# frozenreboot/rplidar_ros2_driver

Measured on AMD Instinct MI355X. Metric: Mpoints/s raw-scan->filtered PointCloud2, higher is better.
Workload: dtype u32/f32

## Files before the change

### rplidar_ros2_driver_amd/csrc/rpl_launch.hpp

```cpp
#pragma once
#include <hip/hip_runtime.h>
#include <stdint.h>

#include "rplgpu.h"
#include "rplgpu_msg.h"
#include "rplgpu_comm.h"
#include "rpl_device.hpp"
#include "rpl_msg.hpp"

namespace rplmsg {
struct Prefix;
}

namespace rpl {

constexpr uint32_t kAscendUnsorted = 0x80000000u;
constexpr uint32_t kRorListedBit = 0x80000000u;
constexpr uint32_t kScanStatusBits =
    RPLGPU_SCAN_ALL_INVALID | RPLGPU_SCAN_CELL_RANGE | RPLGPU_SCAN_TABLE_FULL | RPLGPU_SCAN_OUT_TRUNCATED;
static_assert((kAscendUnsorted & kScanStatusBits) == 0, "internal ascend bit overlaps RPLGPU_SCAN_*");
static_assert((kRorListedBit & kScanStatusBits) == 0, "internal cloud bit overlaps RPLGPU_SCAN_*");
hipError_t launch_ascend(hipStream_t s, void *nodes, uint32_t n_stride, const uint32_t *n_per_scan,
                         uint32_t B, uint32_t *status, uint32_t *need_sort, bool defer_sort = false,
                         uint32_t *sort_stat = nullptr);
hipError_t launch_ascend_sort(hipStream_t s, void *nodes, uint32_t n_stride, const uint32_t *n_per_scan,
                              uint32_t B, uint32_t *status, uint32_t *need_sort,
                              uint32_t *sort_stat = nullptr);
struct LsMsgOut {
  rplmsg::Prefix P;
  uint32_t *msg;
  uint32_t *msg_len;
  int32_t sec;
  uint32_t nanosec;
  double scan_duration;
};
hipError_t launch_laserscan_a(hipStream_t s, const void *nodes, uint32_t n_stride,
                              const uint32_t *n_per_scan, uint32_t B, const KParams &p,
                              const Tables &T, const float *inc_table, const float *rinc_table,
                              bool fast, float *ranges, float *intens, uint32_t *beam_count,
                              uint32_t n_given = 0xFFFFFFFFu, const LsMsgOut *msg_out = nullptr);
hipError_t launch_validate_idx(hipStream_t s, const Tables &T, const float *inc_table,
                               const float *rinc_table, uint32_t max_count,
                               uint32_t *d_mismatches);
hipError_t launch_laserscan_raw(hipStream_t s, const void *nodes, uint32_t n_stride,
                                const uint32_t *n_per_scan, uint32_t B, const KParams &p,
                                float *ranges, float *intens, uint32_t *beam_count);
hipError_t launch_cloud(hipStream_t s, const void *nodes, uint32_t n_stride,
                        const uint32_t *n_per_scan, uint32_t B, const KParams &p, const Tables &T,
                        const uint32_t *keepmask, uint32_t mask_stride, float *xyzi,
                        uint32_t out_stride, uint32_t *n_points, uint32_t *status,
                        const float *motion = nullptr);
enum class ArenaForm : int { kXyzi = 0, kXyi = 1, kCells = 2 };
enum class RorMode : int { kNone = 0, kInside = 1, kListed = 2 };
struct VoxelLaunch {
  const void *nodes = nullptr;
  uint32_t n_stride = 0;
  const uint32_t *n_per_scan = nullptr;
  uint32_t B = 0;
  uint32_t group = 1;
  const float *motion = nullptr, *pose2d = nullptr;
  const uint32_t *keepmask = nullptr;
  uint32_t mask_stride = 0;
  RorMode ror = RorMode::kNone;
  float *xyzi = nullptr;
  uint32_t out_stride = 0;
  float *arena = nullptr;
  uint64_t arena_capacity = 0;
  uint64_t *arena_cursor = nullptr, *scan_start = nullptr;
  ArenaForm form = ArenaForm::kXyzi;
  uint32_t *n_points = nullptr, *status = nullptr;
};
hipError_t launch_cloud_voxel(hipStream_t s, const VoxelLaunch &v, const KParams &p, const Tables &T);
uint32_t voxel_max_workgroups(uint32_t n_cu);
inline uint64_t voxel_store_need(uint32_t group, uint32_t n_stride) {
  const uint64_t s = n_stride < kMaxN ? n_stride : kMaxN;
  return (uint64_t)(group ? group : 1u) * (s + 2u * ((s + 123u) / 124u) + 1u + 528u);
}
hipError_t launch_ror_mask(hipStream_t s, const void *nodes, uint32_t n_stride,
                           const uint32_t *n_per_scan, uint32_t B, const KParams &p,
                           const Tables &T, uint32_t *mask, uint32_t mask_stride,
                           bool listed = false, uint32_t group = 1);
hipError_t launch_validate_div(hipStream_t s, float d, float rd, uint32_t e_lo, uint32_t e_hi,
                               uint32_t *d_mismatches);
hipError_t launch_pack(hipStream_t s, const float *xyzi, uint32_t out_stride,
                       const uint32_t *n_points, uint32_t B, float *packed, uint64_t *offsets);

hipError_t launch_laserscan_to_cloud(hipStream_t s, const float *ranges, const float *intens,
                                     uint32_t n_stride, const uint32_t *beam_count, uint32_t B,
                                     const KParams &p, float *xyzi, uint32_t out_stride,
                                     uint32_t *n_points, uint32_t *status);

hipError_t launch_signal(hipStream_t s, uint32_t *flag, uint32_t seq);
hipError_t launch_stage_in(hipStream_t s, const void *src, void *dst, uint32_t n_words2);
hipError_t launch_pack_meta(hipStream_t s, const unsigned long long *cursor,
                            const unsigned long long *scan_start, const uint32_t *n_points,
                            uint32_t B, unsigned long long slot_points, uint32_t max_scans,
                            uint32_t *meta);
hipError_t launch_unpack_gathered(hipStream_t s, const float *points_all,
                                  unsigned long long slot_points, const uint32_t *meta_all,
                                  uint32_t meta_words, uint32_t world, uint32_t max_scans,
                                  float *packed, unsigned long long *total,
                                  unsigned long long *scan_start_all, uint32_t *n_points_all,
                                  uint32_t *status, uint32_t n_cu, bool xyi = false);
hipError_t launch_merge_cells(hipStream_t s, const void *cells_all, unsigned long long slot_cells,
                              const uint32_t *meta_all, uint32_t meta_words, uint32_t world,
                              uint32_t n_groups, double unit, float *arena,
                              unsigned long long capacity, unsigned long long *cursor,
                              unsigned long long *group_start, uint32_t *n_points, uint32_t *status,
                              uint32_t *scratch, uint32_t n_cu);
hipError_t launch_pack_xyi(hipStream_t s, const float *arena, const unsigned long long *cursor,
                           unsigned long long slot_points, float *slot, uint32_t n_cu);

hipError_t launch_decode(hipStream_t s, int ans, const uint8_t *bytes, uint64_t stream_stride,
                         const uint32_t *frame_off, const uint8_t *gap, const uint32_t *n_frames,
                         uint32_t max_frames, uint32_t B, uint32_t sample_duration_us,
                         const int32_t *state_in, int32_t *state_out, void *nodes,
                         uint32_t node_stride, uint32_t *n_nodes, uint32_t *reset_at,
                         uint32_t reset_stride, uint32_t *n_reset, uint32_t *n_errors,
                         uint32_t *status, uint32_t *sync_at = nullptr, uint32_t sync_stride = 0,
                         uint32_t *n_sync = nullptr, const uint32_t *only = nullptr,
                         bool staged_ok = true, uint32_t *stage_todo = nullptr);
// ... 151 lines not shown
```

### rplidar_ros2_driver_amd/csrc/rpl_voxel.hip

```cpp
#include <algorithm>
#include <cstdlib>
#include <type_traits>

#include "rpl_device.hpp"
#include "rpl_launch.hpp"
#include "rpl_xf.hpp"

namespace rpl {

#ifndef RPL_VOXEL_THREADS
#define RPL_VOXEL_THREADS 1024
#endif
#ifndef RPL_VOXEL_WGS_PER_CU
#define RPL_VOXEL_WGS_PER_CU (RPL_VOXEL_THREADS == 512 ? 2 : 1)
#endif
constexpr int kVB = RPL_VOXEL_THREADS;
constexpr int kVW = kVB / 64;
constexpr int kVWG = RPL_VOXEL_WGS_PER_CU;
constexpr uint32_t kRecCap = kVWG == 2 ? 4096u : 7168u;
constexpr uint32_t kRecPerThread = kRecCap / kVB;
constexpr uint32_t kRowCap = kVWG == 2 ? 1024u : 2u * kVB;
constexpr uint32_t kRowsPerThread = kRowCap / kVB;
constexpr uint32_t kBucketCap = kRecCap + 3u * kRowCap;
constexpr uint32_t kEmptyKey = 0xFFFFFFFFu;
// ... 242 lines not shown
  const u32x4 marker = {kEmptyKey, 0u, 0u, 0u};
  VoxelLds &L = S.L;
  uint4 *const G = S.G;
  const uint32_t lds_rec = (uint32_t)(uintptr_t)&L.rec[0];
  if (base + 1u + total <= kRecCap) {
    if (lane_id() == 0) lds_store128(lds_rec + base * 16u, marker);
#pragma unroll
    for (int j = 0; j < NS; ++j)
      if (__builtin_amdgcn_inverse_ballot_w64(m[j])) lds_store128(lds_rec + pos[j] * 16u, rec[j]);
  } else {
    if (lane_id() == 0) {
      if (base < kRecCap) lds_store128(lds_rec + base * 16u, marker); else glb_store128(G + base, marker);
    }
#pragma unroll
    for (int j = 0; j < NS; ++j) {
      if (__builtin_amdgcn_inverse_ballot_w64(m[j])) {
        if (pos[j] < kRecCap) lds_store128(lds_rec + pos[j] * 16u, rec[j]); else glb_store128(G + pos[j], rec[j]);
      }
    }
  }
  return false;
}

template <int NS>
__device__ __forceinline__ void voxel_block_split(QueueSink &S,
                                                  const bool (&ok)[NS], const uint32_t (&key)[NS],
                                                  const uint32_t (&qx)[NS], const uint32_t (&qy)[NS],
                                                  const uint32_t (&ci)[NS]) {
#pragma unroll
  for (uint32_t cls = 0; cls < 2u; ++cls) {
    bool okc[NS];
    uint32_t keyc[NS], qxc[NS], qyc[NS], cic[NS];
#pragma unroll
    for (int j = 0; j < NS; ++j) {
      okc[j] = ok[j] && (((key[j] >> 16) ^ key[j]) & 1u) == cls;
      keyc[j] = key[j];
      qxc[j] = okc[j] ? qx[j] : 0u;
      qyc[j] = okc[j] ? qy[j] : 0u;
      cic[j] = okc[j] ? ci[j] : 0u;
    }
    voxel_block_pass<true, NS, kPassPlain>(S, okc, keyc, qxc, qyc, cic);
  }
}

__device__ __forceinline__ double run_sum_f64(uint32_t u) {
  double s = (double)u;
  if (u >= 0xF0000000u) s -= 4294967296.0;
  return s;
}

struct VoxelArena {
  float4 *base;
  unsigned long long *cursor;
  unsigned long long capacity;
  unsigned long long *scan_start;
  int xyi;
};
enum : int { kEmitLegacy = 0, kEmitArenaFirst = 1, kEmitCountOnly = 2, kEmitArenaKnown = 3, kEmitArenaTemp = 4 };

template <bool DBG>
struct PhaseClock {
  unsigned long long acc[8] = {0, 0, 0, 0, 0, 0, 0, 0}, mark = 0;
  __device__ __forceinline__ void start() {
    if (DBG) mark = clock64();
  }
  __device__ __forceinline__ void lap(int i) {
    if (DBG) {
      const unsigned long long now = clock64();
      acc[i] += now - mark;
      mark = now;
    }
  }
};

template <bool DBG, bool CELLS>
__device__ __forceinline__ uint32_t voxel_reduce(VoxelLds &L, const KParams &p,
                                                 float4 *__restrict__ out, uint32_t out_stride,
                                                 uint32_t b, uint32_t *ncell_out, int mode,
                                                 const VoxelArena &arena, bool normalised,
                                                 const float4 *out_buffer) {
  PhaseClock<DBG> pc;
  pc.start();
  auto flush_dbg = [&]() {
    if (DBG && p.dbg && threadIdx.x == 0) {
#pragma unroll
      for (int i = 1; i < 8; ++i) atomicAdd(&p.dbg[16 * b + i], pc.acc[i]);
    }
  };
  uint32_t *const rowstart = L.rows, *const rowfill = L.rows + kRowCap;
  uint32_t *cell_keys = p.cell_keys ? p.cell_keys + (out - out_buffer) : nullptr;
  const int vbias = p.vox_bias;
  const uint32_t nrec = L.misc[0];
  if (DBG && p.dbg && threadIdx.x == 0) pc.acc[7] += (unsigned long long)nrec << 40;
  uint4 mine[kRecPerThread];
  uint32_t rmin = 0xFFFFFFFFu, rmax = 0u;
#pragma unroll
  for (int k = 0; k < (int)kRecPerThread; ++k) {
    const uint32_t idx = threadIdx.x + (uint32_t)k * kVB;
    uint4 m = make_uint4(kEmptyKey, 0u, 0u, 0u);
    if ((idx & ~63u) < nrec) {
      const uint4 raw = L.rec[idx];
      const bool ok = idx < nrec && raw.x != kEmptyKey;
      m = raw;
      if (!normalised) {
        uint4 pr;
        pr.y = (uint32_t)__builtin_amdgcn_update_dpp(0, (int)raw.y, 0x138, 0xF, 0xF, false);
// ... 480 lines not shown
  return false;
}

template <bool FAST_DIV, bool SAFE, bool SPLIT, bool DBG, int AHEAD, int RORM = 0>
__device__ __forceinline__ void voxel_stream_dispatch(QueueSink &sink, const KParams &p,
                                                      const float2 *__restrict__ cs,
                                                      const __amdgpu_buffer_rsrc_t rsrc, uint32_t blk0,
                                                      uint32_t blk_end, const ScanSide &sd,
                                                      uint32_t mask_stride, bool use_xf,
                                                      uint32_t q_min16, uint32_t ibfe_off,
                                                      uint32_t ibfe_w, uint32_t &flags,
                                                      unsigned long long *dbg_slot,
                                                      RorSide *rs = nullptr, uint32_t oob_off = 0u) {
  if constexpr (RORM == 1) {
    if (use_xf)
      voxel_stream<FAST_DIV, SAFE, SPLIT, false, true, false, true, AHEAD, true>(
          sink, p, cs, rsrc, blk0, blk_end, nullptr, 0u, sd.xf, q_min16, ibfe_off, ibfe_w, flags, nullptr, rs, oob_off);
    else if (q_min16)
      voxel_stream<FAST_DIV, SAFE, SPLIT, false, true, false, false, AHEAD, true>(
          sink, p, cs, rsrc, blk0, blk_end, nullptr, 0u, sd.xf, q_min16, ibfe_off, ibfe_w, flags, nullptr, rs, oob_off);
    else
      voxel_stream<FAST_DIV, SAFE, SPLIT, false, false, false, false, AHEAD, true>(
          sink, p, cs, rsrc, blk0, blk_end, nullptr, 0u, sd.xf, q_min16, ibfe_off, ibfe_w, flags, nullptr, rs, oob_off);
    return;
  }
#define RPL_VS(HQ, HM, XFB)                                                                         \
  voxel_stream<FAST_DIV, SAFE, SPLIT, DBG, HQ, HM, XFB, AHEAD>(sink, p, cs, rsrc, blk0, blk_end, \
                                                                     sd.ror_bits, mask_stride, sd.xf, \
                                                                     q_min16, ibfe_off, ibfe_w, flags, \
                                                                     dbg_slot)
  if constexpr (RORM == 2) {
    if (use_xf) RPL_VS(true, true, true);
    else RPL_VS(true, true, false);
    return;
  }
  if (use_xf) {
    if (sd.ror_bits) RPL_VS(true, true, true);
    else RPL_VS(true, false, true);
  } else if (sd.ror_bits) RPL_VS(true, true, false);
  else if (q_min16) RPL_VS(true, false, false);
  else RPL_VS(false, false, false);
#undef RPL_VS
}

template <bool DBG, int RORM = 0, bool CELLS = false, class FirstBand>
__device__ __forceinline__ void voxel_work_loop(VoxelLds &L, const KParams &p, const Tables &T,
                                                uint4 *__restrict__ G, float4 *__restrict__ xyzi,
                                                uint32_t out_stride, uint32_t *__restrict__ n_points,
                                                uint32_t *__restrict__ status, uint32_t B,
                                                uint32_t item0, const VoxelArena &arena,
                                                FirstBand &&first_band) {
  if (threadIdx.x < 256) L.rcp[threadIdx.x] = T.rcp[threadIdx.x];
  if constexpr (RORM == 2) B = min(B, (uint32_t)__builtin_amdgcn_readfirstlane((int)T.redo[0]));
  for (uint32_t bl = blockIdx.x; bl < B;) {
  const uint32_t b = RORM == 2 ? T.redo[4u + bl] : item0 + bl;
  bool abandoned = false;
  float4 *out = arena.base ? arena.base : xyzi + (size_t)b * out_stride;
  int emit_mode = arena.base ? kEmitArenaFirst : kEmitLegacy;
  unsigned long long arena_at = 0ull;

  if (threadIdx.x < 16) L.misc[threadIdx.x] = 0u;
  if (threadIdx.x == 0) {
    L.band_lo[0] = 0u;
    L.band_hi[0] = 0xFFFFFFFEu;
    L.misc[3] = 1u;
    L.tmp[28] = 0u;
    L.tmp[29] = 0u;
  }
  __syncthreads();

  uint32_t flags = 0;
  PhaseClock<DBG> pc;
  pc.start();

  bool first = true;
  bool leave_single_band_mode_early = false;
  bool from_store = false;
  uint32_t n_all = 0;
  while (true) {
    const uint32_t sp = L.misc[3];
    if (sp == 0) break;
    const uint32_t klo = L.band_lo[sp - 1], khi = L.band_hi[sp - 1];
    __syncthreads();
    if (threadIdx.x == 0) {
      L.misc[0] = 0u;
      L.misc[2] = 0u;
      L.misc[3] = sp - 1;
      L.misc[4] = 0xFFFFFFFFu;
      L.misc[5] = 0u;
      L.misc[8] = 0xFFFFFFFFu;
      L.misc[9] = 0u;
    }
    for (uint32_t t = threadIdx.x; t < kRowCap; t += kVB) L.rows[t] = 0u;
    __syncthreads();

    if (first) {
      abandoned = first_band(b, bl, flags);
      first = false;
      asm volatile("s_waitcnt vmcnt(0) lgkmcnt(0)" ::: "memory");
      __syncthreads();
      if (RORM == 1 && abandoned) {
        if (threadIdx.x == 0) {
          T.redo[4u + atomicAdd(&T.redo[0], 1u)] = b;
          n_points[b] = 0u;
          if (status) status[b] = kRorListedBit;
          if (arena.base) arena.scan_start[b] = 0ull;
// ... 245 lines not shown
        L.misc[7] = 0u;
      }
      __syncthreads();
      arena_at = ((unsigned long long)L.tmp[29] << 32) | L.tmp[28];
      out = arena.base + arena_at;
      emit_mode = kEmitArenaKnown;
    }
    if (emit_mode == kEmitArenaTemp && L.misc[3] == 0u) {
      const uint32_t total = L.misc[7];
      if (threadIdx.x == 0) {
        const unsigned long long at = atomicAdd(arena.cursor, (unsigned long long)total);
        L.tmp[28] = (uint32_t)at;
        L.tmp[29] = (uint32_t)(at >> 32);
      }
      __syncthreads();
      arena_at = ((unsigned long long)L.tmp[29] << 32) | L.tmp[28];
      const unsigned long long room = arena_at >= arena.capacity ? 0ull : arena.capacity - arena_at;
      const uint32_t ncopy = (uint32_t)min((unsigned long long)total, room);
      const float4 *src = reinterpret_cast<const float4 *>(G + T.voxel_store_recs);
      if (arena.xyi) {
        float *dst = reinterpret_cast<float *>(arena.base) + 3u * (size_t)arena_at;
        for (uint32_t i = threadIdx.x; i < ncopy; i += kVB) {
          const float4 v = src[i];
          dst[3u * i] = v.x;
          dst[3u * i + 1u] = v.y;
          dst[3u * i + 2u] = v.w;
        }
      } else {
        float4 *dst = arena.base + arena_at;
        for (uint32_t i = threadIdx.x; i < ncopy; i += kVB) dst[i] = src[i];
      }
    }
  }
  if (DBG && p.dbg && threadIdx.x == 0) {
    atomicAdd(&p.dbg[16 * b], pc.acc[0]);
    atomicAdd(&p.dbg[16 * b + 2], pc.acc[2]);
  }

  if (flags) atomicOr(&L.misc[1], flags);
  __syncthreads();
  if (threadIdx.x == 0 && !abandoned) {
    const uint32_t total = L.misc[7];
    if (arena.base) {
      const unsigned long long room = arena_at >= arena.capacity ? 0ull : arena.capacity - arena_at;
      const uint32_t kept = (uint32_t)min((unsigned long long)total, room);
      arena.scan_start[b] = arena_at;
      n_points[b] = kept;
      if (status) status[b] = L.misc[1] | (kept < total ? RPLGPU_SCAN_OUT_TRUNCATED : 0u);
    } else {
      n_points[b] = min(total, out_stride);
      if (status) status[b] = L.misc[1] | ((total > out_stride) ? RPLGPU_SCAN_OUT_TRUNCATED : 0u);
    }
  }
  if (RORM != 2 && B <= gridDim.x) return;
  if (threadIdx.x == 0) L.tmp[31] = gridDim.x + atomicAdd(&T.work_ctr[0], 1u);
  __syncthreads();
  bl = L.tmp[31];
  __syncthreads();
  }
}

template <bool FAST_DIV, bool SAFE, bool DBG, bool SPLIT, int RORM = 0>
__global__ __launch_bounds__(kVB) __attribute__((amdgpu_waves_per_eu(kVB * kVWG / 256, kVB * kVWG / 256))) void k_cloud_voxel(
    const uint2 *__restrict__ nodes, uint32_t n_stride, const uint32_t *__restrict__ n_per_scan,
    KParams p, Tables T, const uint32_t *__restrict__ keepmask, uint32_t mask_stride,
    float4 *__restrict__ xyzi, uint32_t out_stride, uint32_t *__restrict__ n_points,
    uint32_t *__restrict__ status, uint32_t B, VoxelArena arena, uint4 *__restrict__ store,
    uint32_t group, uint32_t n_scans, const float *__restrict__ motion,
    const float *__restrict__ pose2d) {
  __shared__ VoxelLds L;
  uint4 *G = store + (size_t)blockIdx.x * 2u * T.voxel_store_recs;
  const float2 *cs = p.inverted ? T.cs_inv : T.cs;
  const uint32_t ishift = p.is_new_protocol ? 0u : 2u;
  const uint32_t ibfe_off = 16u + ishift, ibfe_w = 0xFFu >> ishift;
  const uint32_t q_min16 = p.clip_enable ? (min(p.q_min, 256u) << 16) : 0u;
  const bool use_xf = (group > 1u) || motion || pose2d;
  __shared__ RorSide Rs;
  auto phase_s = [&](uint32_t b, uint32_t, uint32_t &flags) -> bool {
    QueueSink sink{L, G};
    const uint32_t s_lo = b * group, s_hi = min(n_scans, s_lo + group);
    for (uint32_t sc = s_lo; sc < s_hi; ++sc) {
      const uint32_t n = (uint32_t)__builtin_amdgcn_readfirstlane(
          (int)min(n_per_scan[sc], min(n_stride, kMaxN)));
      const uint2 *scan = nodes + (size_t)sc * n_stride;
      const __amdgpu_buffer_rsrc_t scan_rsrc =
          __builtin_amdgcn_make_buffer_rsrc((void *)scan, 0, (int)(n * 8u), 0x00020000);
      const ScanSide sd = scan_side(sc, keepmask, mask_stride, motion, pose2d, T.scan_t0);
      const uint32_t blk0 = (uint32_t)__builtin_amdgcn_readfirstlane((int)wave_id());
      if constexpr (RORM == 1) {
        if (threadIdx.x == 0) { Rs.n_todo = 0u; Rs.n_todo2 = 0u; }
        __syncthreads();
        voxel_stream_dispatch<FAST_DIV, SAFE, SPLIT, false, RPL_VOXEL_AHEAD, 1>(
            sink, p, cs, scan_rsrc, blk0, (n + 123u) / 124u, sd, 0u, use_xf, q_min16, ibfe_off, ibfe_w, flags,
            nullptr, &Rs, (n * 8u + 15u) & ~15u);
        asm volatile("s_waitcnt vmcnt(0) lgkmcnt(0)" ::: "memory");
        __syncthreads();
        bool clutter;
        if (use_xf)
          clutter = ror_resolve<FAST_DIV, SAFE, true>(sink, Rs, p, cs, scan, n, sd.xf, q_min16, ibfe_off, ibfe_w, flags);
        else
          clutter = ror_resolve<FAST_DIV, SAFE, false>(sink, Rs, p, cs, scan, n, sd.xf, q_min16, ibfe_off, ibfe_w, flags);
        if (clutter) return true;
        __syncthreads();
      } else {
        voxel_stream_dispatch<FAST_DIV, SAFE, SPLIT, DBG, RPL_VOXEL_AHEAD, RORM>(
            sink, p, cs, scan_rsrc, blk0, (n + 127u) >> 7, sd, mask_stride, use_xf, q_min16, ibfe_off,
            ibfe_w, flags, (DBG && p.dbg) ? p.dbg + 16 * b : nullptr);
      }
    }
    return false;
  };
  voxel_work_loop<DBG, RORM, SPLIT || RORM != 0>(L, p, T, G, xyzi, out_stride, n_points, status, B, 0u, arena, phase_s);
}

__global__ __launch_bounds__(256) void k_validate_div(float d, float rd, uint32_t e_lo,
                                                      uint32_t e_hi, uint32_t *mismatches) {
  const uint64_t per_exp = 1ull << 23;
  const uint64_t total = (uint64_t)(e_hi - e_lo + 1) * per_exp;
  uint32_t bad = 0;
  for (uint64_t t = (uint64_t)blockIdx.x * blockDim.x + threadIdx.x; t < total;
       t += (uint64_t)gridDim.x * blockDim.x) {
    uint32_t bits = ((uint32_t)(e_lo + (uint32_t)(t >> 23)) << 23) | (uint32_t)(t & (per_exp - 1));
    float a = __uint_as_float(bits);
    float na = __uint_as_float(bits | 0x80000000u);
    const f2 q2 = div_by2(f2{a, na}, d, rd);
    bad += (__float_as_uint(q2.x) != __float_as_uint(a / d));
    bad += (__float_as_uint(q2.y) != __float_as_uint(na / d));
    bad += (__float_as_uint(div_by(a, d, rd)) != __float_as_uint(a / d));
  }
  if (blockIdx.x == 0 && threadIdx.x == 0) {
    bad += (div_by(0.0f, d, rd) != 0.0f);
    bad += (div_by(-0.0f, d, rd) != 0.0f);
  }
  if (bad) atomicAdd(mismatches, bad);
}

hipError_t launch_validate_div(hipStream_t s, float d, float rd, uint32_t e_lo, uint32_t e_hi,
                               uint32_t *d_mismatches) {
  hipLaunchKernelGGL(k_validate_div, dim3(256 * 16), dim3(256), 0, s, d, rd, e_lo, e_hi,
                     d_mismatches);
  return hipGetLastError();
}

uint32_t voxel_max_workgroups(uint32_t n_cu) { return (uint32_t)kVWG * (n_cu ? n_cu : 256u); }


hipError_t launch_cloud_voxel(hipStream_t s, const VoxelLaunch &v, const KParams &p, const Tables &T) {
  static_assert(sizeof(unsigned long long) == sizeof(uint64_t), "64-bit cursor");
  uint32_t B = v.B, group = v.group;
  const bool ror = v.ror != RorMode::kNone, listed = v.ror == RorMode::kListed;
  if (B == 0) return hipSuccess;
  if (ror && (!p.fast_div || !T.redo || p.dbg)) return hipErrorInvalidValue;
  if (listed && !v.keepmask) return hipErrorInvalidValue;
  if (v.form == ArenaForm::kCells && !ror && (p.dbg || !T.voxel_split)) return hipErrorInvalidValue;
  if (group == 0) group = 1;
  group = std::min(group, B);
  const uint32_t n_scans = B;
  B = (B + group - 1u) / group;
  if (!T.voxel_store || T.voxel_store_wgs == 0) return hipErrorInvalidValue;
  if (voxel_store_need(group, v.n_stride) > T.voxel_store_recs) return hipErrorInvalidValue;
  VoxelArena ar;
  ar.base = (float4 *)v.arena;
  ar.cursor = reinterpret_cast<unsigned long long *>(v.arena_cursor);
  ar.capacity = v.arena_capacity;
  ar.scan_start = reinterpret_cast<unsigned long long *>(v.scan_start);
  ar.xyi = v.arena ? (int)v.form : 0;
  if (kVWG == 2 && group > 1) return hipErrorInvalidValue;
  uint32_t grid = std::min<uint32_t>(std::min<uint32_t>(B, voxel_max_workgroups(T.n_cu)),
                                     T.voxel_store_wgs);
  if (const char *e = std::getenv("RPLGPU_VOXEL_GRID")) {
    const long g = std::atol(e);
    if (g > 0) grid = std::min<uint32_t>(grid, (uint32_t)g);
  }
  const bool with_stats = T.voxel_stats && T.voxel_stats_host && B >= 64u && !listed;
  Tables Tk = T;
  if (!with_stats) Tk.voxel_stats = nullptr;
  if (with_stats)
    if (hipError_t e = hipMemsetAsync(T.voxel_stats, 0, 16, s); e != hipSuccess) return e;
  if (grid < B || listed)
    if (hipError_t e = hipMemsetAsync(T.work_ctr, 0, 4, s); e != hipSuccess) return e;
#define RPL_LAUNCH_VOXEL(FD, SF, DB, SP)                                                          \
  hipLaunchKernelGGL((k_cloud_voxel<FD, SF, DB, SP>), dim3(grid), dim3(kVB), 0, s, (const uint2 *)v.nodes, \
                     v.n_stride, v.n_per_scan, p, Tk, v.keepmask, v.mask_stride, (float4 *)v.xyzi, v.out_stride, \
                     v.n_points, v.status, B, ar, (uint4 *)T.voxel_store, group, n_scans, v.motion, v.pose2d)
#define RPL_LAUNCH_VOXEL_SF(FD, DB, SP)                                                           \
  do {                                                                                             \
    if (p.cell_range_safe) RPL_LAUNCH_VOXEL(FD, true, DB, SP); else RPL_LAUNCH_VOXEL(FD, false, DB, SP); \
  } while (0)
#define RPL_LAUNCH_VOXEL_ROR(SF, SP, RM)                                                          \
  hipLaunchKernelGGL((k_cloud_voxel<true, SF, false, SP, RM>), dim3(grid), dim3(kVB), 0, s,         \
                     (const uint2 *)v.nodes, v.n_stride, v.n_per_scan, p, Tk, v.keepmask, v.mask_stride, \
                     (float4 *)v.xyzi, v.out_stride, v.n_points, v.status, B, ar, (uint4 *)T.voxel_store, \
                     group, n_scans, v.motion, v.pose2d)
#define RPL_LAUNCH_VOXEL_ROR_SF(SP, RM)                                                           \
  do {                                                                                             \
    if (p.cell_range_safe) RPL_LAUNCH_VOXEL_ROR(true, SP, RM); else RPL_LAUNCH_VOXEL_ROR(false, SP, RM); \
  } while (0)
  if (v.ror == RorMode::kInside) {
    if (T.voxel_split) RPL_LAUNCH_VOXEL_ROR_SF(true, 1); else RPL_LAUNCH_VOXEL_ROR_SF(false, 1);
  } else if (listed) {
    if (T.voxel_split) RPL_LAUNCH_VOXEL_ROR_SF(true, 2); else RPL_LAUNCH_VOXEL_ROR_SF(false, 2);
  } else
  if (p.dbg) {
    if (p.fast_div) RPL_LAUNCH_VOXEL_SF(true, true, false); else RPL_LAUNCH_VOXEL_SF(false, true, false);
  } else if (T.voxel_split) {
    if (p.fast_div) RPL_LAUNCH_VOXEL_SF(true, false, true); else RPL_LAUNCH_VOXEL_SF(false, false, true);
  } else {
    if (p.fast_div) RPL_LAUNCH_VOXEL_SF(true, false, false); else RPL_LAUNCH_VOXEL_SF(false, false, false);
  }
#undef RPL_LAUNCH_VOXEL_SF
#undef RPL_LAUNCH_VOXEL
#undef RPL_LAUNCH_VOXEL_ROR_SF
#undef RPL_LAUNCH_VOXEL_ROR
  if (with_stats) {
    if (hipError_t e = hipMemcpyAsync(T.voxel_stats_host, T.voxel_stats, 16, hipMemcpyDeviceToHost, s);
        e != hipSuccess)
      return e;
  }
  return hipGetLastError();
}

}
```

### rplidar_ros2_driver_amd/csrc/rplgpu_api.hip

```cpp
#include <hip/hip_runtime.h>
#include <dlfcn.h>

#include <algorithm>
#include <cmath>
#include <cstdio>
#include <cstdlib>
#include <cstring>
#include <limits>
#include <new>
#include <string>
#include <thread>
#include <vector>

#include "rplgpu.h"
#include "rplgpu_msg.h"
#include "rpl_launch.hpp"
#include "rpl_msg.hpp"
#include "rpl_comm_layout.hpp"
#include "rpl_cells.hpp"

struct VoxelBatchId {
  const void *nodes = nullptr;
  uint32_t n_stride = 0, B = 0, group = 0;
  bool operator==(const VoxelBatchId &o) const {
    return nodes == o.nodes && n_stride == o.n_stride && B == o.B && group == o.group;
  }
};

struct rplgpu_ctx {
  int device = -1;
  hipStream_t own_stream = nullptr;
  hipStream_t stream = nullptr;
  uint32_t max_n = 0, max_b = 0;
  float *d_angle = nullptr, *d_angle_inv = nullptr, *d_inc = nullptr, *d_rinc = nullptr;
  float2 *d_cs = nullptr, *d_cs_inv = nullptr;
  double *d_rcp = nullptr;
  unsigned char *h_pin = nullptr;
  unsigned char *d_pin = nullptr;
  bool zero_copy = true;
  bool spin_sync = true;
  size_t flag_off = 0;
  uint32_t scan_seq = 0;
  struct Pinned { unsigned char *host, *dev; size_t bytes; };
  std::vector<Pinned> pinned;
  unsigned char *d_nodes = nullptr, *d_out = nullptr;
  uint32_t *d_rormask = nullptr;
  uint32_t *d_redo = nullptr;
  int32_t ror_fused = 1;
  uint32_t *d_need_sort = nullptr;
  uint32_t need_sort_cap = 0;
  uint32_t *d_small = nullptr;
  bool div4000_ok = false;
  float leaf_checked = 0.0f;
  bool leaf_ok = false;
  bool idx_checked = false, idx_ok = false;
  uint32_t force_ieee = 0;
  unsigned long long *dbg = nullptr;
  uint32_t *cell_keys = nullptr;
  const float *scan_t0 = nullptr;
  unsigned long long *h_vstats = nullptr;
  uint32_t stats_group = 1;
  bool stats_valid = false;
  VoxelBatchId stats_id;
  struct VoxelDecision { VoxelBatchId id; bool split = false; bool valid = false; };
  VoxelDecision decisions[8];
  uint32_t next_decision = 0;
  int32_t last_split = 0;
  uint32_t n_cu = 0;
  void *d_vstore = nullptr;
  int32_t force_split = -1;
  bool dec_stage = true;
  uint32_t vstore_wgs = 0;
  uint32_t vstore_recs = 0;
  uint32_t *d_merge = nullptr;
  size_t merge_cap = 0;
  unsigned long long *d_mkeys = nullptr;
  size_t mkeys_cap = 0;
  bool mkeys_clean = true;
  float2 *d_medges = nullptr;
  size_t medges_cap = 0;
  bool mspec_valid = false;
  rplgpu_scan_merge_t mspec;
  rpl::MergeK mspec_k;
  unsigned char *d_dec = nullptr;
  size_t dec_cap = 0;
  unsigned char *d_scans = nullptr;
  size_t scans_cap = 0;
  uint32_t *d_dec_todo = nullptr;
  size_t dec_todo_cap = 0;
  bool check_ptrs = true;
  void *comm = nullptr;
  int32_t comm_rank = 0, comm_world = 0;
  hipStream_t xstream = nullptr;
  hipEvent_t ev_main = nullptr, ev_x[4] = {nullptr, nullptr, nullptr, nullptr};
  uint32_t n_exchanges = 0;
  std::string err;
};

struct rplgpu_nccl_id_t {
  char internal[128];
};

namespace {

constexpr uint32_t kMaskStride = rpl::kMaxN / 32u;
constexpr size_t kTail = 64;

constexpr size_t round64(size_t v) { return (v + 63u) & ~(size_t)63u; }
constexpr size_t stage_out_off(size_t max_n) { return round64(max_n * 8) + kTail; }
constexpr size_t stage_flag_off(size_t max_n) { return stage_out_off(max_n) + round64(max_n * 16) + kTail; }
constexpr size_t stage_bytes(size_t max_n) { return stage_flag_off(max_n) + kTail; }

thread_local std::string g_create_err;
// ... 78 lines not shown
}

bool voxel_split_for(rplgpu_ctx *c, const void *d_nodes, uint32_t n_stride, uint32_t B, uint32_t group) {
  group = std::max(1u, std::min(group, std::max(B, 1u)));
  const VoxelBatchId id{d_nodes, n_stride, B, group};
  const bool with_stats = c->h_vstats && (B + group - 1u) / group >= 64u;
  auto find = [&](const VoxelBatchId &k) -> rplgpu_ctx::VoxelDecision * {
    for (auto &d : c->decisions)
      if (d.valid && d.id == k) return &d;
    return nullptr;
  };
  if (c->h_vstats && c->stats_valid) {
    const unsigned long long entries = __atomic_load_n(&c->h_vstats[0], __ATOMIC_RELAXED);
    const unsigned long long items = __atomic_load_n(&c->h_vstats[1], __ATOMIC_RELAXED);
    const uint32_t g = c->stats_group;
    if (items != 0 && entries <= items * g * 70000ull) {
      rplgpu_ctx::VoxelDecision *d = find(c->stats_id);
      if (!d) {
        d = &c->decisions[c->next_decision];
        c->next_decision = (c->next_decision + 1u) % (uint32_t)(sizeof(c->decisions) / sizeof(c->decisions[0]));
        d->id = c->stats_id;
        d->split = false;
        d->valid = true;
      }
      const unsigned long long avg = entries / (items * g);
      if (!d->split && avg > 6500ull) d->split = true;
      else if (d->split && avg < 4000ull) d->split = false;
    }
  }
  const rplgpu_ctx::VoxelDecision *mine = find(id);
  const bool split = mine ? mine->split : false;
  if (with_stats) {
    c->stats_id = id;
    c->stats_valid = true;
    c->stats_group = group;
  }
  c->last_split = (c->force_split >= 0 ? c->force_split != 0 : split) ? 1 : 0;
  return c->last_split != 0;
}

rpl::Tables tables_of(rplgpu_ctx *c) {
  rpl::Tables t;
  t.angle = c->d_angle;
  t.angle_inv = c->d_angle_inv;
  t.cs = c->d_cs;
  t.cs_inv = c->d_cs_inv;
  t.rcp = c->d_rcp;
  t.work_ctr = c->d_small + 16;
  t.n_cu = c->n_cu;
  t.voxel_store = c->d_vstore;
  t.voxel_store_wgs = c->vstore_wgs;
  t.voxel_store_recs = c->vstore_recs;
  t.voxel_stats = reinterpret_cast<unsigned long long *>(c->d_small + 24);
  t.voxel_stats_host = c->h_vstats;
  t.voxel_split = c->force_split > 0 ? 1 : 0;
  t.scan_t0 = c->scan_t0;
  t.redo = c->d_redo;
  return t;
}

void build_tables(std::vector<float> &angle, std::vector<float> &angle_inv,
                  std::vector<float2> &cs, std::vector<float2> &cs_inv, std::vector<float> &inc,
                  std::vector<float> &rinc) {
  angle.resize(65536);
  angle_inv.resize(65536);
  cs.resize(65536);
  cs_inv.resize(65536);
  for (int q = 0; q < 65536; ++q) {
    uint16_t angle_z_q14 = (uint16_t)q;
    float angle_deg = angle_z_q14 * 90.0f / 16384.0f;
    float angle_rad = angle_deg * (M_PI / 180.0f);
    if (angle_rad < 0.0f) angle_rad += 2.0f * M_PI;
    if (angle_rad >= 2.0f * M_PI) angle_rad -= 2.0f * M_PI;
    float inv = (2.0f * M_PI) - angle_rad;
    if (inv >= 2.0f * M_PI) inv -= 2.0f * M_PI;
    angle[q] = angle_rad;
    angle_inv[q] = inv;
    cs[q] = make_float2((float)std::cos((double)angle_rad), (float)std::sin((double)angle_rad));
    cs_inv[q] = make_float2((float)std::cos((double)inv), (float)std::sin((double)inv));
  }
  inc.resize(rpl::kMaxN + 1);
  inc[0] = 0.0f;
  for (uint32_t c = 1; c <= rpl::kMaxN; ++c)
    inc[c] = static_cast<float>((2.0 * M_PI) / static_cast<double>(c));
  rinc.resize(rpl::kMaxN + 1);
  rinc[0] = 0.0f;
  for (uint32_t c = 1; c <= rpl::kMaxN; ++c) rinc[c] = 1.0f / inc[c];
}

template <class T>
int32_t upload(rplgpu_ctx *c, T **dst, const std::vector<T> &src) {
  RPL_HIP(c, hipMalloc((void **)dst, src.size() * sizeof(T)));
  RPL_HIP(c, hipMemcpy(*dst, src.data(), src.size() * sizeof(T), hipMemcpyHostToDevice));
  return RPLGPU_OK;
}

void comm_teardown(rplgpu_ctx *c);

void free_ctx(rplgpu_ctx *c) {
  if (!c) return;
  if (c->device >= 0) (void)hipSetDevice(c->device);
  comm_teardown(c);
  if (c->d_angle) (void)hipFree(c->d_angle);
  if (c->d_angle_inv) (void)hipFree(c->d_angle_inv);
  if (c->d_inc) (void)hipFree(c->d_inc);
  if (c->d_rinc) (void)hipFree(c->d_rinc);
  if (c->d_cs) (void)hipFree(c->d_cs);
// ... 226 lines not shown
  if (const char *e = std::getenv("RPLGPU_CHECK_POINTERS")) c->check_ptrs = std::atoi(e) != 0;
  auto fail = [&](int32_t code) {
    g_create_err = c->err;
    free_ctx(c);
    return code;
  };
  if (hipStreamCreateWithFlags(&c->own_stream, hipStreamNonBlocking) != hipSuccess)
    return fail(RPLGPU_ERR_HIP);
  c->stream = c->own_stream;

  std::vector<float> angle, angle_inv, inc, rinc;
  std::vector<float2> cs, cs_inv;
  build_tables(angle, angle_inv, cs, cs_inv, inc, rinc);
  for (int q = 1; q < 65536; ++q) {
    if (!(angle[q] > angle[q - 1])) {
      c->err = "angle table not strictly increasing";
      return fail(RPLGPU_ERR_INVALID_ARG);
    }
  }
  std::vector<double> rcp(rpl::kMaxN + 1);
  rcp[0] = 0.0;
  for (uint32_t k = 1; k <= rpl::kMaxN; ++k) rcp[k] = 1.0 / static_cast<double>(k);
  int32_t rc;
  if ((rc = upload(c, &c->d_rcp, rcp)) || (rc = upload(c, &c->d_angle, angle)) || (rc = upload(c, &c->d_angle_inv, angle_inv)) ||
      (rc = upload(c, &c->d_cs, cs)) || (rc = upload(c, &c->d_cs_inv, cs_inv)) ||
      (rc = upload(c, &c->d_inc, inc)) || (rc = upload(c, &c->d_rinc, rinc)))
    return fail(rc);

  const size_t n = c->max_n;
  c->flag_off = stage_flag_off(n);
  if (hipHostMalloc((void **)&c->h_pin, stage_bytes(n), hipHostMallocDefault) != hipSuccess ||
      hipMalloc((void **)&c->d_nodes, n * 8 + kTail) != hipSuccess ||
      hipMalloc((void **)&c->d_out, n * 16 + kTail) != hipSuccess ||
      hipMalloc((void **)&c->d_small, 128) != hipSuccess ||
      hipMalloc((void **)&c->d_need_sort, ((size_t)c->max_b + 1u) * 4u) != hipSuccess ||
      hipMalloc((void **)&c->d_rormask, (size_t)c->max_b * kMaskStride * 4u) != hipSuccess ||
      hipMalloc((void **)&c->d_redo, ((size_t)c->max_b + 4u) * 4u) != hipSuccess) {
    c->err = "staging allocation failed";
    return fail(RPLGPU_ERR_HIP);
  }
  c->need_sort_cap = c->max_b;
  if (hipMemset(c->d_need_sort, 0, 4) != hipSuccess || hipMemset(c->d_redo, 0, 4) != hipSuccess) {
    c->err = "staging allocation failed";
    return fail(RPLGPU_ERR_HIP);
  }
  c->vstore_wgs = std::min<uint32_t>(c->max_b, rpl::voxel_max_workgroups(c->n_cu));
  c->vstore_recs = (uint32_t)rpl::voxel_store_need(1u, rpl::kMaxN);
  if (hipMalloc(&c->d_vstore, (size_t)c->vstore_wgs * c->vstore_recs * 32u) != hipSuccess) {
    c->err = "record store allocation failed";
    return fail(RPLGPU_ERR_HIP);
  }
  if (hipHostMalloc((void **)&c->h_vstats, 16, hipHostMallocDefault) == hipSuccess) {
    c->h_vstats[0] = c->h_vstats[1] = 0ull;
  } else {
    c->h_vstats = nullptr;
    (void)hipGetLastError();
  }
  if (hipHostGetDevicePointer((void **)&c->d_pin, c->h_pin, 0) != hipSuccess) c->d_pin = nullptr;
  if (const char *e = std::getenv("RPLGPU_ZERO_COPY")) c->zero_copy = std::atoi(e) != 0;
  if (!c->d_pin) c->zero_copy = false;
  if (const char *e = std::getenv("RPLGPU_SPIN_SYNC")) c->spin_sync = std::atoi(e) != 0;
  if (const char *e = std::getenv("RPLGPU_DEC_STAGE")) c->dec_stage = std::atoi(e) != 0;
  if (const char *e = std::getenv("RPLGPU_VOXEL_SPLIT")) c->force_split = std::atoi(e) != 0;
  if (const char *e = std::getenv("RPLGPU_ROR_FUSED")) c->ror_fused = std::atoi(e) != 0;
  std::memset(c->h_pin + c->flag_off, 0, kTail);
  if (hipMemset(c->d_small, 0, 128) != hipSuccess) {
    c->err = "staging clear failed";
    return fail(RPLGPU_ERR_HIP);
  }
  if (validate_divisor(c, 4000.0f, 127, 159, &c->div4000_ok) != RPLGPU_OK) return fail(RPLGPU_ERR_HIP);
  if (validate_divisor(c, 0.05f, 27, 167, &c->leaf_ok) != RPLGPU_OK) return fail(RPLGPU_ERR_HIP);
  c->leaf_checked = 0.05f;
  *out = c;
  return RPLGPU_OK;
}

int32_t rplgpu_destroy(rplgpu_handle_t h) {
  if (!h) return RPLGPU_ERR_INVALID_ARG;
  (void)hipSetDevice(h->device);
  (void)hipStreamSynchronize(h->stream);
  free_ctx(h);
  return RPLGPU_OK;
}

const char *rplgpu_last_error(rplgpu_handle_t h) {
  if (!h) return g_create_err.c_str();
  return h->err.c_str();
}

int32_t rplgpu_set_stream(rplgpu_handle_t h, void *hip_stream) {
  if (!h) return RPLGPU_ERR_INVALID_ARG;
  hipStream_t next = hip_stream ? (hipStream_t)hip_stream : h->own_stream;
  if (next != h->stream) {
    RPL_HIP(h, hipSetDevice(h->device));
    RPL_HIP(h, hipStreamSynchronize(h->stream));
  }
  h->stream = next;
  return RPLGPU_OK;
}

int32_t rplgpu_set_cell_key_output(rplgpu_handle_t h, uint32_t *d_cell_keys) {
  if (!h) return RPLGPU_ERR_INVALID_ARG;
  if (d_cell_keys && !device_readable(h, d_cell_keys, "d_cell_keys")) return RPLGPU_ERR_INVALID_ARG;
  h->cell_keys = d_cell_keys;
  return RPLGPU_OK;
}
// ... 124 lines not shown

static bool ror_runs_inside(const rplgpu_ctx *h, const CloudRequest &req, const rplgpu_params_t &p,
                            const rpl::KParams &kp) {
  return !req.force_two_kernels && h->ror_fused && p.voxel_enable && kp.fast_div && !kp.dbg;
}

static int32_t prepare_cloud(rplgpu_handle_t h, const rplgpu_node_t *d_nodes, uint32_t n_stride,
                             const uint32_t *d_n_per_scan, uint32_t B, const rplgpu_params_t *p,
                             const CloudRequest &req, CloudPlan *plan) {
  if (p->ror_enable && !(p->ror_radius > 0.0f && p->ror_radius <= 1.0e6f)) {
    h->err = "ror_radius must be in (0, 1e6] m";
    return RPLGPU_ERR_INVALID_ARG;
  }
  if (p->voxel_enable && !(p->voxel_leaf >= 1e-6f && p->voxel_leaf <= 1024.0f)) {
    h->err = "voxel_leaf must be in [1e-6, 1024] m";
    return RPLGPU_ERR_INVALID_ARG;
  }
  RPL_HIP(h, hipSetDevice(h->device));
  plan->kp = to_kparams(*p);
  rpl::KParams &kp = plan->kp;
  if (p->voxel_enable) {
    if (h->leaf_checked != p->voxel_leaf) {
      int32_t vrc = validate_divisor(h, p->voxel_leaf, 27, 167, &h->leaf_ok);
      if (vrc) return vrc;
      h->leaf_checked = p->voxel_leaf;
    }
    kp.fast_div = (use_fast_d4000(h) && use_fast_leaf(h)) ? 1 : 0;
  }
  kp.fast_d4000 = use_fast_d4000(h) ? 1 : 0;
  kp.dbg = h->dbg;
  kp.cell_keys = h->cell_keys;
  plan->T = tables_of(h);
  if (p->ror_enable) {
    plan->ror_inside = ror_runs_inside(h, req, *p, kp);
    if (!plan->ror_inside) {
      RPL_HIP(h, rpl::launch_ror_mask(h->stream, d_nodes, n_stride, d_n_per_scan, B, kp, plan->T,
                                      h->d_rormask, kMaskStride));
      plan->mask = h->d_rormask;
    }
  }
  if (req.cells) {
    kp.cell_keys = nullptr;
    kp.dbg = nullptr;
  }
  if (p->voxel_enable) {
    plan->T.voxel_split = voxel_split_for(h, d_nodes, n_stride, B, req.group) ? 1 : 0;
    if (req.cells && !plan->ror_inside) plan->T.voxel_split = 1;
  }
  return RPLGPU_OK;
}

static int32_t run_voxel(rplgpu_handle_t h, const CloudPlan &plan, rpl::VoxelLaunch v,
                         bool defer_listed = false) {
  if (v.arena) RPL_HIP(h, hipMemsetAsync(v.arena_cursor, 0, 8, h->stream));
  v.keepmask = plan.mask;
  v.mask_stride = kMaskStride;
  if (plan.ror_inside) {
    RPL_HIP(h, hipMemsetAsync(h->d_redo, 0, 4, h->stream));
    v.ror = rpl::RorMode::kInside;
  }
  RPL_HIP(h, rpl::launch_cloud_voxel(h->stream, v, plan.kp, plan.T));
  if (!plan.ror_inside || defer_listed) return RPLGPU_OK;
  RPL_HIP(h, rpl::launch_ror_mask(h->stream, v.nodes, v.n_stride, v.n_per_scan, v.B, plan.kp, plan.T,
                                  h->d_rormask, kMaskStride, true, std::max(1u, std::min(v.group, v.B))));
  v.keepmask = h->d_rormask;
  v.ror = rpl::RorMode::kListed;
  RPL_HIP(h, rpl::launch_cloud_voxel(h->stream, v, plan.kp, plan.T));
  return RPLGPU_OK;
}

static int32_t cloud_arena_impl(rplgpu_handle_t h, const rplgpu_node_t *d_nodes, uint32_t n_stride,
                               const uint32_t *d_n_per_scan, uint32_t B, const rplgpu_params_t *p,
                               float *d_arena, uint64_t arena_capacity, uint64_t *d_cursor,
                               uint64_t *d_scan_start, uint32_t *d_n_points, uint32_t *d_status,
                               bool xyi) {
  int32_t rc = check_batch(h, d_nodes, n_stride, d_n_per_scan, B);
  if (rc) return rc;
  if (!p || !d_arena || !d_cursor || !d_scan_start || !d_n_points) return RPLGPU_ERR_INVALID_ARG;
  if (!p->voxel_enable) {
    h->err = "rplgpu_cloud_arena_dev needs voxel_enable";
    return RPLGPU_ERR_INVALID_ARG;
  }
  CloudPlan plan;
  if ((rc = prepare_cloud(h, d_nodes, n_stride, d_n_per_scan, B, p, CloudRequest{}, &plan))) return rc;
  rpl::VoxelLaunch v{d_nodes, n_stride, d_n_per_scan, B};
  v.arena = d_arena;
  v.arena_capacity = arena_capacity;
  v.arena_cursor = d_cursor;
  v.scan_start = d_scan_start;
  v.form = xyi ? rpl::ArenaForm::kXyi : rpl::ArenaForm::kXyzi;
  v.n_points = d_n_points;
  v.status = d_status;
  return run_voxel(h, plan, v);
}

int32_t rplgpu_cloud_arena_dev(rplgpu_handle_t h, const rplgpu_node_t *d_nodes, uint32_t n_stride,
                               const uint32_t *d_n_per_scan, uint32_t B, const rplgpu_params_t *p,
                               float *d_arena, uint64_t arena_capacity, uint64_t *d_cursor,
                               uint64_t *d_scan_start, uint32_t *d_n_points, uint32_t *d_status) {
  return cloud_arena_impl(h, d_nodes, n_stride, d_n_per_scan, B, p, d_arena, arena_capacity, d_cursor,
                          d_scan_start, d_n_points, d_status, false);
}

int32_t rplgpu_cloud_arena_xyi_dev(rplgpu_handle_t h, const rplgpu_node_t *d_nodes,
                                   uint32_t n_stride, const uint32_t *d_n_per_scan, uint32_t B,
                                   const rplgpu_params_t *p, float *d_slot, uint64_t slot_points,
                                   uint64_t *d_cursor, uint64_t *d_scan_start, uint32_t *d_n_points,
                                   uint32_t *d_status) {
  return cloud_arena_impl(h, d_nodes, n_stride, d_n_per_scan, B, p, d_slot, slot_points, d_cursor,
                          d_scan_start, d_n_points, d_status, true);
}

static int32_t fused_impl(rplgpu_handle_t h, const rplgpu_node_t *d_nodes, uint32_t n_stride,
                          const uint32_t *d_n_per_scan, uint32_t B, uint32_t group,
                          const rplgpu_params_t *p, const float *d_motion, const float *d_pose2d,
                          float *d_arena, uint64_t arena_capacity, uint64_t *d_cursor,
                          uint64_t *d_group_start, uint32_t *d_n_points, uint32_t *d_status,
                          bool cells) {
  int32_t rc = check_batch(h, d_nodes, n_stride, d_n_per_scan, B);
  if (rc) return rc;
// ... 2641 lines not shown
```

Before: 293,900.

## Self-reset voxel counters in-kernel and write stats to host-mapped memory

The last workgroup to finish (tracked by an atomic ticket) now publishes the arena cursor, copies voxel stats straight to host-mapped memory, and zeroes the work counters. This removes the per-launch hipMemsetAsync calls for the work counter, stats and arena cursor, plus the device-to-host stats copy, leaving fewer stream operations per batch. It relies on the kernel always leaving counters clean and on a dirty flag to re-clear them after an error. It also adds a completion atomic and fences at the end of every workgroup.

```diff
diff --git a/rplidar_ros2_driver_amd/csrc/rpl_launch.hpp b/rplidar_ros2_driver_amd/csrc/rpl_launch.hpp
--- a/rplidar_ros2_driver_amd/csrc/rpl_launch.hpp
+++ b/rplidar_ros2_driver_amd/csrc/rpl_launch.hpp
@@ -67,6 +67,7 @@
   float *arena = nullptr;
   uint64_t arena_capacity = 0;
   uint64_t *arena_cursor = nullptr, *scan_start = nullptr;
+  bool reserve_inside = false;
   ArenaForm form = ArenaForm::kXyzi;
   uint32_t *n_points = nullptr, *status = nullptr;
 };
diff --git a/rplidar_ros2_driver_amd/csrc/rpl_voxel.hip b/rplidar_ros2_driver_amd/csrc/rpl_voxel.hip
--- a/rplidar_ros2_driver_amd/csrc/rpl_voxel.hip
+++ b/rplidar_ros2_driver_amd/csrc/rpl_voxel.hip
@@ -318,6 +318,7 @@
 struct VoxelArena {
   float4 *base;
   unsigned long long *cursor;
+  unsigned long long *publish;
   unsigned long long capacity;
   unsigned long long *scan_start;
   int xyi;
@@ -904,6 +905,7 @@
                                                 FirstBand &&first_band) {
   if (threadIdx.x < 256) L.rcp[threadIdx.x] = T.rcp[threadIdx.x];
   if constexpr (RORM == 2) B = min(B, (uint32_t)__builtin_amdgcn_readfirstlane((int)T.redo[0]));
+  const bool queued = RORM == 2 || B > gridDim.x;
   for (uint32_t bl = blockIdx.x; bl < B;) {
   const uint32_t b = RORM == 2 ? T.redo[4u + bl] : item0 + bl;
   bool abandoned = false;
@@ -1255,11 +1257,26 @@
       if (status) status[b] = L.misc[1] | ((total > out_stride) ? RPLGPU_SCAN_OUT_TRUNCATED : 0u);
     }
   }
-  if (RORM != 2 && B <= gridDim.x) return;
+  if (!queued) break;
   if (threadIdx.x == 0) L.tmp[31] = gridDim.x + atomicAdd(&T.work_ctr[0], 1u);
   __syncthreads();
   bl = L.tmp[31];
   __syncthreads();
+  }
+  if (threadIdx.x == 0) {
+    __threadfence();
+    if (atomicAdd(&T.work_ctr[1], 1u) == gridDim.x - 1u) {
+      __threadfence();
+      if (arena.publish) *arena.publish = atomicExch(arena.cursor, 0ull);
+      if (T.voxel_stats) {
+        const unsigned long long entries = atomicExch(&T.voxel_stats[0], 0ull);
+        const unsigned long long items = atomicExch(&T.voxel_stats[1], 0ull);
+        __hip_atomic_store(&T.voxel_stats_host[0], entries, __ATOMIC_RELAXED, __HIP_MEMORY_SCOPE_SYSTEM);
+        __hip_atomic_store(&T.voxel_stats_host[1], items, __ATOMIC_RELAXED, __HIP_MEMORY_SCOPE_SYSTEM);
+      }
+      atomicExch(&T.work_ctr[0], 0u);
+      atomicExch(&T.work_ctr[1], 0u);
+    }
   }
 }
 
@@ -1365,6 +1382,11 @@
   VoxelArena ar;
   ar.base = (float4 *)v.arena;
   ar.cursor = reinterpret_cast<unsigned long long *>(v.arena_cursor);
+  ar.publish = nullptr;
+  if (v.arena && v.reserve_inside) {
+    ar.cursor = reinterpret_cast<unsigned long long *>(T.work_ctr + 2);
+    ar.publish = reinterpret_cast<unsigned long long *>(v.arena_cursor);
+  }
   ar.capacity = v.arena_capacity;
   ar.scan_start = reinterpret_cast<unsigned long long *>(v.scan_start);
   ar.xyi = v.arena ? (int)v.form : 0;
@@ -1378,10 +1400,6 @@
   const bool with_stats = T.voxel_stats && T.voxel_stats_host && B >= 64u && !listed;
   Tables Tk = T;
   if (!with_stats) Tk.voxel_stats = nullptr;
-  if (with_stats)
-    if (hipError_t e = hipMemsetAsync(T.voxel_stats, 0, 16, s); e != hipSuccess) return e;
-  if (grid < B || listed)
-    if (hipError_t e = hipMemsetAsync(T.work_ctr, 0, 4, s); e != hipSuccess) return e;
 #define RPL_LAUNCH_VOXEL(FD, SF, DB, SP)                                                          \
   hipLaunchKernelGGL((k_cloud_voxel<FD, SF, DB, SP>), dim3(grid), dim3(kVB), 0, s, (const uint2 *)v.nodes, \
                      v.n_stride, v.n_per_scan, p, Tk, v.keepmask, v.mask_stride, (float4 *)v.xyzi, v.out_stride, \
@@ -1415,11 +1433,6 @@
 #undef RPL_LAUNCH_VOXEL
 #undef RPL_LAUNCH_VOXEL_ROR_SF
 #undef RPL_LAUNCH_VOXEL_ROR
-  if (with_stats) {
-    if (hipError_t e = hipMemcpyAsync(T.voxel_stats_host, T.voxel_stats, 16, hipMemcpyDeviceToHost, s);
-        e != hipSuccess)
-      return e;
-  }
   return hipGetLastError();
 }
 
diff --git a/rplidar_ros2_driver_amd/csrc/rplgpu_api.hip b/rplidar_ros2_driver_amd/csrc/rplgpu_api.hip
--- a/rplidar_ros2_driver_amd/csrc/rplgpu_api.hip
+++ b/rplidar_ros2_driver_amd/csrc/rplgpu_api.hip
@@ -59,6 +59,8 @@
   uint32_t *cell_keys = nullptr;
   const float *scan_t0 = nullptr;
   unsigned long long *h_vstats = nullptr;
+  unsigned long long *d_vstats = nullptr;
+  bool voxel_words_dirty = true;
   uint32_t stats_group = 1;
   bool stats_valid = false;
   VoxelBatchId stats_id;
@@ -243,7 +245,7 @@
   t.voxel_store_wgs = c->vstore_wgs;
   t.voxel_store_recs = c->vstore_recs;
   t.voxel_stats = reinterpret_cast<unsigned long long *>(c->d_small + 24);
-  t.voxel_stats_host = c->h_vstats;
+  t.voxel_stats_host = c->d_vstats;
   t.voxel_split = c->force_split > 0 ? 1 : 0;
   t.scan_t0 = c->scan_t0;
   t.redo = c->d_redo;
@@ -576,6 +578,11 @@
   }
   if (hipHostMalloc((void **)&c->h_vstats, 16, hipHostMallocDefault) == hipSuccess) {
     c->h_vstats[0] = c->h_vstats[1] = 0ull;
+    if (hipHostGetDevicePointer((void **)&c->d_vstats, c->h_vstats, 0) != hipSuccess || !c->d_vstats) {
+      (void)hipHostFree(c->h_vstats);
+      c->h_vstats = c->d_vstats = nullptr;
+      (void)hipGetLastError();
+    }
   } else {
     c->h_vstats = nullptr;
     (void)hipGetLastError();
@@ -806,7 +813,13 @@
 
 static int32_t run_voxel(rplgpu_handle_t h, const CloudPlan &plan, rpl::VoxelLaunch v,
                          bool defer_listed = false) {
-  if (v.arena) RPL_HIP(h, hipMemsetAsync(v.arena_cursor, 0, 8, h->stream));
+  if (h->voxel_words_dirty) {
+    RPL_HIP(h, hipMemsetAsync(h->d_small + 16, 0, 16, h->stream));
+    RPL_HIP(h, hipMemsetAsync(h->d_small + 24, 0, 16, h->stream));
+  }
+  h->voxel_words_dirty = true;
+  v.reserve_inside = v.arena && !plan.ror_inside && v.B != 0;
+  if (v.arena && !v.reserve_inside) RPL_HIP(h, hipMemsetAsync(v.arena_cursor, 0, 8, h->stream));
   v.keepmask = plan.mask;
   v.mask_stride = kMaskStride;
   if (plan.ror_inside) {
@@ -814,12 +827,16 @@
     v.ror = rpl::RorMode::kInside;
   }
   RPL_HIP(h, rpl::launch_cloud_voxel(h->stream, v, plan.kp, plan.T));
-  if (!plan.ror_inside || defer_listed) return RPLGPU_OK;
+  if (!plan.ror_inside || defer_listed) {
+    h->voxel_words_dirty = false;
+    return RPLGPU_OK;
+  }
   RPL_HIP(h, rpl::launch_ror_mask(h->stream, v.nodes, v.n_stride, v.n_per_scan, v.B, plan.kp, plan.T,
                                   h->d_rormask, kMaskStride, true, std::max(1u, std::min(v.group, v.B))));
   v.keepmask = h->d_rormask;
   v.ror = rpl::RorMode::kListed;
   RPL_HIP(h, rpl::launch_cloud_voxel(h->stream, v, plan.kp, plan.T));
+  h->voxel_words_dirty = false;
   return RPLGPU_OK;
 }
 
```

After: 294,200 (median of 3 runs). About the same (+0.1%).
